# JasonHopeSpace/panda

Measured on AMD Instinct MI355X. Metric: MSM points/s (BN254, 2^24), higher is better.
Workload: dtype u32; 1 GPU; BN254 MSM 2^24 points per GPU, Jacobian output, bases and scalars resident in HBM; curve=bn254, log_points_per_gpu=24, exchange=none

## Files before the change

### panda_amd/csrc/msm_sort.hip

```cpp
#include <algorithm>
#include <atomic>
#include <cmath>

#include "fe29.h"
#include "msm_sort.h"

using namespace panda29;

namespace {

constexpr unsigned SORT_TILE = 8192;
constexpr unsigned MAX_PARTS = 1024;
constexpr unsigned SORT_THREADS = 1024;
constexpr unsigned BS_CHUNK = 8192;

template <class Code>
struct CodeTraits;
template <>
struct CodeTraits<uint16_t> {
    static constexpr u32 ZERO = 0x7fffu;
    static constexpr u32 MAG = 0x7fffu;
    static constexpr int SIGN = 15;
};
template <>
struct CodeTraits<u32> {
    static constexpr u32 ZERO = 0x7fffffffu;
    static constexpr u32 MAG = 0x7fffffffu;
    static constexpr int SIGN = 31;
};

template <int WORDS>
__device__ __forceinline__ void load_words(u32 *dst, const u32 *src)
{
    static_assert(WORDS % 4 == 0, "vector loads");
    const uint4 *s4 = reinterpret_cast<const uint4 *>(src);
#pragma unroll
    for (int i = 0; i < WORDS / 4; i++) {
        uint4 v = s4[i];
        dst[4 * i] = v.x;
        dst[4 * i + 1] = v.y;
        dst[4 * i + 2] = v.z;
        dst[4 * i + 3] = v.w;
    }
}

__device__ __forceinline__ void check_samples(const panda::SampleCheck &sc)
{
    int differs = 0;
    for (unsigned t = threadIdx.x >> 2; t < panda::REG_SAMPLES; t += blockDim.x >> 2) {
        const u64 row = panda::sample_row(t, sc.n);
        for (unsigned k = threadIdx.x & 3u; k < sc.row_words; k += 4) differs |= sc.samples[t * sc.row_words + k] != sc.wire[row * sc.row_words + k];
    }
    differs = __syncthreads_or(differs);
    if (threadIdx.x == 0) {
        *sc.flag_dev = differs ? 1u : 0u;
        if (differs) *sc.flag_host = 1u;
    }
}

struct DigitsBatch {
    unsigned log_n, prefix_bit;
};

__device__ __forceinline__ void stage_plan(u32 *wlo, const panda::WindowPlan &plan)
{
    for (unsigned k = threadIdx.x; k < plan.W; k += blockDim.x) wlo[k] = plan.lo[k] | ((u32)plan.width[k] << 16);
}

template <int L, class CT, class Fn>
__device__ __forceinline__ void for_each_digit(const u32 *s, const u32 *wlo, unsigned W, u32 prefix, Fn f)
{
    u32 carry = 0;
    unsigned k = 0;
    auto digit = [&](u32 raw, unsigned c) {
        const u32 half = 1u << (c - 1), full = 1u << c;
        raw += carry;
        u32 code;
        if (raw >= half) {
            u32 mag = full - raw;
            carry = 1;
            code = mag ? ((1u << CT::SIGN) | prefix | (mag - 1)) : CT::ZERO;
        } else {
            carry = 0;
            code = raw ? (prefix | (raw - 1)) : CT::ZERO;
        }
        f(k, code);
    };
#pragma unroll
    for (int m = 0; m < L; m++) {
        const u64 v = s[m] | ((u64)s[m + 1] << 32);
        while (k < W) {
            const u32 e = __builtin_amdgcn_readfirstlane(wlo[k]);
            const unsigned lo = e & 0xffffu, c = e >> 16;
            if ((lo >> 5) != (unsigned)m) break;
            digit((u32)(v >> (lo & 31)) & ((1u << c) - 1), c);
            k++;
        }
    }
    for (; k < W; k++) digit(0, __builtin_amdgcn_readfirstlane(wlo[k]) >> 16);
}

template <class Fr, class Code, bool BATCH = false>
__global__ void __launch_bounds__(256) k_digits(const u32 *__restrict__ scalars, Code *__restrict__ dig, u64 n, panda::WindowPlan plan, panda::SampleCheck sc,
                                                DigitsBatch bg)
{
    typedef CodeTraits<Code> CT;
    constexpr int L = Fr::L;
    __shared__ u32 wlo[panda::MAX_WINDOWS];
    if (blockIdx.x == 0 && sc.wire) check_samples(sc);
    stage_plan(wlo, plan);
    __syncthreads();
    u64 i = (u64)blockIdx.x * blockDim.x + threadIdx.x;
    if (i >= n) return;
    u32 w[L], s[L + 1];
    load_words<L>(w, scalars + i * L);
    fe_wire_to_canonical<Fr>(s, w);
    s[L] = 0;
    const u32 prefix = BATCH ? (u32)(i >> bg.log_n) << bg.prefix_bit : 0u;
    for_each_digit<L, CT>(s, wlo, plan.W, prefix, [&](unsigned k, u32 code) { dig[(u64)k * n + i] = (Code)code; });
}

struct DigitsHistGeom {
    unsigned lo_bits, H, tiles;
};

template <class Fr, class Code, bool BATCH = false>
__global__ void __launch_bounds__(1024) k_digits_hist(const u32 *__restrict__ scalars, Code *__restrict__ dig, u32 *__restrict__ tile_hist, u64 n,
                                                     panda::WindowPlan plan, DigitsHistGeom g, panda::SampleCheck sc, DigitsBatch bg)
{
    typedef CodeTraits<Code> CT;
    constexpr int L = Fr::L;
    extern __shared__ u32 hist[];
    __shared__ u32 wlo[panda::MAX_WINDOWS];
    if (blockIdx.x == 0 && sc.wire) check_samples(sc);
    const unsigned tile = blockIdx.x, tid = threadIdx.x;
    const unsigned WH = plan.W * g.H, threads = blockDim.x;
    for (unsigned i = tid; i < WH; i += threads) hist[i] = 0;
    stage_plan(wlo, plan);
    __syncthreads();
    const u64 begin = (u64)tile * SORT_TILE, end = begin + SORT_TILE < n ? begin + SORT_TILE : n;
    u32 w[L];
    if (begin + tid < end) load_words<L>(w, scalars + (begin + tid) * L);
    for (u64 i = begin + tid; i < end; i += threads) {
        u32 s[L + 1];
        fe_wire_to_canonical<Fr>(s, w);
        if (i + threads < end) load_words<L>(w, scalars + (i + threads) * L);
        s[L] = 0;
        const u32 prefix = BATCH ? (u32)(i >> bg.log_n) << bg.prefix_bit : 0u;
        for_each_digit<L, CT>(s, wlo, plan.W, prefix, [&](unsigned k, u32 code) {
            dig[(u64)k * n + i] = (Code)code;
            if (code != CT::ZERO) atomicAdd(&hist[k * g.H + ((code & CT::MAG) >> g.lo_bits)], 1u);
        });
    }
    __syncthreads();
    for (unsigned i = tid; i < WH; i += threads) {
        const unsigned k = i / g.H, h = i - k * g.H;
        tile_hist[((u64)k * g.tiles + tile) * g.H + h] = hist[i];
    }
}

template <class Code, class Fn>
__device__ __forceinline__ void for_each_code(const Code *__restrict__ dw, u64 begin, u64 end, Fn f)
{
    constexpr unsigned PER = 16 / sizeof(Code);
    if (reinterpret_cast<uintptr_t>(dw + begin) & 15) {
        for (u64 a = begin + threadIdx.x; a < end; a += blockDim.x) f(a, (u32)dw[a]);
        return;
    }
    for (u64 a = begin + (u64)threadIdx.x * PER; a < end; a += (u64)blockDim.x * PER) {
        const uint4 v = *reinterpret_cast<const uint4 *>(dw + a);
        const u32 wv[4] = {v.x, v.y, v.z, v.w};
#pragma unroll
        for (unsigned j = 0; j < PER; j++) {
            const u32 code = sizeof(Code) == 2 ? (wv[j >> 1] >> (16 * (j & 1))) & 0xffffu : wv[j];
            if (a + j < end) f(a + j, code);
        }
    }
}


struct SortGeom {
    unsigned log_n, lo_bits, H, tiles;
    u32 row0;
};

template <class Code>
__global__ void __launch_bounds__(256) k_part_hist(const Code *__restrict__ dig, u32 *__restrict__ tile_hist, SortGeom g)
{
    typedef CodeTraits<Code> CT;
    __shared__ u32 h[MAX_PARTS];
    const unsigned w = blockIdx.y, tile = blockIdx.x, tid = threadIdx.x;
    for (unsigned i = tid; i < g.H; i += 256) h[i] = 0;
    __syncthreads();
    const u64 n = (u64)1 << g.log_n;
    const Code *dw = dig + ((u64)w << g.log_n);
    const u64 begin = (u64)tile * SORT_TILE, end = begin + SORT_TILE < n ? begin + SORT_TILE : n;
    for_each_code<Code>(dw, begin, end, [&](u64, u32 code) {
        if (code != CT::ZERO) atomicAdd(&h[(code & CT::MAG) >> g.lo_bits], 1u);
    });
    __syncthreads();
    u32 *out = tile_hist + ((u64)w * g.tiles + tile) * g.H;
    for (unsigned i = tid; i < g.H; i += 256) out[i] = h[i];
}

__global__ void __launch_bounds__(1024) k_part_scan_cols(const u32 *__restrict__ tile_hist, u32 *__restrict__ tile_pref, u32 *__restrict__ totals, SortGeom g)
{
    const unsigned w = blockIdx.y, lane = threadIdx.x & 63, h = blockIdx.x * 16 + (threadIdx.x >> 6);
    if (h >= g.H) return;
    const u64 col = (u64)w * g.tiles * g.H + h;
    u32 run = 0;
    for (unsigned t0 = 0; t0 < g.tiles; t0 += 64) {
        const unsigned tile = t0 + lane;
        u32 v = tile < g.tiles ? tile_hist[col + (u64)tile * g.H] : 0;
        u32 inc = v;
        for (unsigned d = 1; d < 64; d <<= 1) {
            u32 up = __shfl_up(inc, d, 64);
            if (lane >= d) inc += up;
        }
        if (tile < g.tiles) tile_pref[col + (u64)tile * g.H] = run + inc - v;
        run += __shfl(inc, 63, 64);
    }
    if (lane == 0) totals[(u64)w * g.H + h] = run;
}

__device__ __forceinline__ u32 block_inclusive_scan(u32 v, u32 *wsum)
{
    const unsigned lane = threadIdx.x & 63u, wave = threadIdx.x >> 6;
    for (unsigned d = 1; d < 64; d <<= 1) {
        const u32 up = __shfl_up(v, d, 64);
        if (lane >= d) v += up;
    }
    if (lane == 63) wsum[wave] = v;
    __syncthreads();
    for (unsigned w = 0; w < wave; w++) v += wsum[w];
    return v;
}

__global__ void __launch_bounds__(1024) k_part_offsets(const u32 *__restrict__ totals, u32 *__restrict__ part_off, SortGeom g)
{
    __shared__ u32 wsum[16];
    const unsigned w = blockIdx.x, t = threadIdx.x;
    const u32 mine = t < g.H ? totals[(u64)w * g.H + t] : 0;
    const u32 inc = block_inclusive_scan(mine, wsum);
    if (t < g.H) part_off[(u64)w * (g.H + 1) + t] = inc - mine;
    if (t == 1023) part_off[(u64)w * (g.H + 1) + g.H] = inc;
}

template <class Code, unsigned THREADS>
struct TileCodes {
    static constexpr unsigned PER = 16 / sizeof(Code), LOADS = SORT_TILE / (THREADS * PER);
    static_assert(LOADS * THREADS * PER == SORT_TILE, "whole loads");
    uint4 v[LOADS];
    bool vec;
    __device__ __forceinline__ void load(const Code *__restrict__ dw, u64 begin, u64 end)
    {
        vec = !(reinterpret_cast<uintptr_t>(dw + begin) & 15);
        if (!vec) return;
#pragma unroll
        for (unsigned q = 0; q < LOADS; q++) {
            const u64 a = begin + ((u64)q * THREADS + threadIdx.x) * PER;
            v[q] = a < end ? *reinterpret_cast<const uint4 *>(dw + a) : uint4{0, 0, 0, 0};
        }
    }
    __device__ __forceinline__ u32 code(unsigned q, unsigned j) const
    {
        const u32 wv[4] = {v[q].x, v[q].y, v[q].z, v[q].w};
        return sizeof(Code) == 2 ? (wv[j >> 1] >> (16 * (j & 1))) & 0xffffu : wv[j];
    }
    template <class Rank, class Place>
    __device__ __forceinline__ void rank_and_place(const Code *__restrict__ dw, u64 begin, u64 end, Rank rank, Place place) const
    {
        if (!vec) {
            for_each_code<Code>(dw, begin, end, [&](u64 i, u32 c) { place(i, c, rank(i, c)); });
            return;
        }
        u32 slot[LOADS * PER];
#pragma unroll
        for (unsigned q = 0; q < LOADS; q++) {
            const u64 a = begin + ((u64)q * THREADS + threadIdx.x) * PER;
#pragma unroll
            for (unsigned j = 0; j < PER; j++)
                if (a + j < end) slot[q * PER + j] = rank(a + j, code(q, j));
        }
#pragma unroll
        for (unsigned q = 0; q < LOADS; q++) {
            const u64 a = begin + ((u64)q * THREADS + threadIdx.x) * PER;
#pragma unroll
            for (unsigned j = 0; j < PER; j++)
                if (a + j < end) place(a + j, code(q, j), slot[q * PER + j]);
        }
    }
};

template <class Code, class Word>
__global__ void __launch_bounds__(SORT_THREADS) k_part_scatter(const Code *__restrict__ dig, const u32 *__restrict__ tile_hist, const u32 *__restrict__ tile_pref,
                                                      const u32 *__restrict__ part_off, Word *__restrict__ p1, SortGeom g)
{
    typedef CodeTraits<Code> CT;
    static_assert(MAX_PARTS <= SORT_THREADS, "a partition counter per thread");
    __shared__ u32 lcur[MAX_PARTS];
    __shared__ u32 delta[MAX_PARTS];
    __shared__ Word words[SORT_TILE];
    __shared__ uint16_t parts_of[SORT_TILE];
    __shared__ u32 wsum[SORT_THREADS / 64];
    const unsigned w = blockIdx.y, tile = blockIdx.x, tid = threadIdx.x;
    const u64 row = ((u64)w * g.tiles + tile) * g.H;
    const u32 *po = part_off + (u64)w * (g.H + 1);
    const u64 n = (u64)1 << g.log_n;
    const Code *dw = dig + ((u64)w << g.log_n);
    Word *pw = p1 + ((u64)w << g.log_n);
    const u64 begin = (u64)tile * SORT_TILE, end = begin + SORT_TILE < n ? begin + SORT_TILE : n;
    const u32 lo_mask = (1u << g.lo_bits) - 1;
    TileCodes<Code, SORT_THREADS> codes;
    codes.load(dw, begin, end);
    const u32 count = tid < g.H ? tile_hist[row + tid] : 0;
    const u32 gbase = tid < g.H ? po[tid] + tile_pref[row + tid] : 0;
    const u32 lstart = block_inclusive_scan(count, wsum) - count;
    if (tid < g.H) {
        lcur[tid] = lstart;
        delta[tid] = gbase - lstart;
    }
    __syncthreads();
    codes.rank_and_place(
        dw, begin, end, [&](u64, u32 code) -> u32 { return code == CT::ZERO ? 0u : atomicAdd(&lcur[(code & CT::MAG) >> g.lo_bits], 1u); },
        [&](u64 i, u32 code, u32 slot) {
            if (code == CT::ZERO) return;
            u32 b = code & CT::MAG, h = b >> g.lo_bits;
            words[slot] = ((Word)(b & lo_mask) << (g.log_n + 1)) | (Word)(((code >> CT::SIGN) << g.log_n) | (u32)i);
            parts_of[slot] = (uint16_t)h;
        });
    __syncthreads();
    const u32 total = lcur[g.H - 1];
    for (u32 j = tid; j < total; j += SORT_THREADS) pw[delta[parts_of[j]] + j] = words[j];
}

template <class Code>
__global__ void __launch_bounds__(SORT_THREADS) k1_scatter_split(const Code *__restrict__ dig, const u32 *__restrict__ tile_hist, const u32 *__restrict__ tile_pref,
                                                        const u32 *__restrict__ part_off, u32 *__restrict__ p1_lo, unsigned char *__restrict__ p1_hi, SortGeom g,
                                                        unsigned b3)
{
    typedef CodeTraits<Code> CT;
    static_assert(MAX_PARTS <= SORT_THREADS, "a partition counter per thread");
    __shared__ u32 lcur[MAX_PARTS];
    __shared__ u32 delta[MAX_PARTS];
    __shared__ u32 words[SORT_TILE];
    __shared__ u32 meta[SORT_TILE];
    __shared__ u32 wsum[SORT_THREADS / 64];
    const unsigned w = blockIdx.y, tile = blockIdx.x, tid = threadIdx.x, lane = tid & 63u;
    const u64 row = ((u64)w * g.tiles + tile) * g.H;
    const u32 *po = part_off + (u64)w * (g.H + 1);
    const u64 n = (u64)1 << g.log_n;
    const Code *dw = dig + ((u64)w << g.log_n);
    u32 *plo = p1_lo + ((u64)w << g.log_n);
    unsigned char *phi = p1_hi + ((u64)w << g.log_n);
    const u64 begin = (u64)tile * SORT_TILE, end = begin + SORT_TILE < n ? begin + SORT_TILE : n;
    const u32 b3_mask = (1u << b3) - 1, b2_mask = (1u << (g.lo_bits - b3)) - 1;
    TileCodes<Code, SORT_THREADS> codes;
    codes.load(dw, begin, end);
    const u32 count = tid < g.H ? tile_hist[row + tid] : 0;
    const u32 gbase = tid < g.H ? po[tid] + tile_pref[row + tid] : 0;
    const u32 lstart = block_inclusive_scan(count, wsum) - count;
    if (tid < g.H) {
        lcur[tid] = lstart;
        delta[tid] = gbase - lstart;
    }
    __syncthreads();
    codes.rank_and_place(
        dw, begin, end, [&](u64, u32 code) -> u32 { return code == CT::ZERO ? 0u : atomicAdd(&lcur[(code & CT::MAG) >> g.lo_bits], 1u); },
        [&](u64 i, u32 code, u32 slot) {
            if (code == CT::ZERO) return;
            u32 b = code & CT::MAG, h = b >> g.lo_bits;
            words[slot] = ((b & b3_mask) << (g.log_n + 1)) | ((code >> CT::SIGN) << g.log_n) | (u32)i;
            meta[slot] = (h << 8) | ((b >> b3) & b2_mask);
        });
    __syncthreads();
    const u32 total = lcur[g.H - 1];
    for (u32 base = 0; base < total; base += SORT_THREADS) {
        const u32 j = base + tid;
        const bool valid = j < total;
        const u32 m = valid ? meta[j] : ~0u;
        const u32 h = m >> 8;
        u32 dst = 0;
        if (valid) {
            dst = delta[h] + j;
            plo[dst] = words[j];
        }
        const u32 m1 = __shfl_down(m, 1, 64), m2 = __shfl_down(m, 2, 64), m3 = __shfl_down(m, 3, 64);
        const bool lead = valid && lane <= 60 && !(reinterpret_cast<uintptr_t>(phi + dst) & 3) && (m1 >> 8) == h && (m2 >> 8) == h && (m3 >> 8) == h;
        const u64 leaders = __ballot(lead);
        const bool covered = (((leaders << 1) | (leaders << 2) | (leaders << 3)) >> lane) & 1;
        if (lead)
            *reinterpret_cast<u32 *>(phi + dst) = (m & 0xffu) | ((m1 & 0xffu) << 8) | ((m2 & 0xffu) << 16) | (m3 << 24);
        else if (valid && !covered)
            phi[dst] = (unsigned char)m;
    }
}

__device__ __forceinline__ void scan128_inclusive(u32 *cnt, u32 *carry )
{
    const unsigned tid = threadIdx.x, lane = tid & 63u;
    u32 v = tid < 128 ? cnt[tid] : 0;
    if (tid < 128) {
        for (unsigned d = 1; d < 64; d <<= 1) {
            const u32 up = __shfl_up(v, d, 64);
            if (lane >= d) v += up;
        }
        if (tid == 63) *carry = v;
    }
    __syncthreads();
    if (tid >= 64 && tid < 128) v += *carry;
    if (tid < 128) cnt[tid] = v;
    __syncthreads();
}

__global__ void __launch_bounds__(SORT_THREADS) k_bucket_sort(const u32 *__restrict__ p1, const u32 *__restrict__ part_off, u32 *__restrict__ off,
                                                     u32 *__restrict__ sorted, SortGeom g, unsigned NB)
{
    __shared__ u32 cnt[128], cur[128], lstart[128], lcur[128], scan_carry;
    __shared__ u32 words[BS_CHUNK];
    __shared__ unsigned char lo_of[BS_CHUNK];
    const unsigned w = blockIdx.y, h = blockIdx.x, tid = threadIdx.x;
    const unsigned L = 1u << g.lo_bits;
    const u32 ps = part_off[(u64)w * (g.H + 1) + h], pe = part_off[(u64)w * (g.H + 1) + h + 1];
    const u32 *pw = p1 + ((u64)w << g.log_n);
    u32 *sw = sorted + ((u64)w << g.log_n);
    const unsigned shift = g.log_n + 1;
    if (tid < 128) cnt[tid] = 0;
    __syncthreads();
    for (u32 j = ps + tid; j < pe; j += SORT_THREADS) atomicAdd(&cnt[pw[j] >> shift], 1u);
    __syncthreads();
    u32 mine = tid < 128 ? cnt[tid] : 0;
    scan128_inclusive(cnt, &scan_carry);
    if (tid < L) {
        u32 start = ps + cnt[tid] - mine;
        cur[tid] = start;
        off[(u64)w * (NB + 1) + ((u64)h << g.lo_bits) + tid] = start;
    }
    if (h == g.H - 1 && tid == 0) off[(u64)w * (NB + 1) + NB] = pe;
    __syncthreads();
    const u32 id_mask = (1u << g.log_n) - 1;
    for (u32 cbeg = ps; cbeg < pe; cbeg += BS_CHUNK) {
        const u32 cend = min(cbeg + BS_CHUNK, pe);
        if (tid < 128) {
            lstart[tid] = 0;
            lcur[tid] = 0;
        }
        __syncthreads();
        for (u32 j = cbeg + tid; j < cend; j += SORT_THREADS) atomicAdd(&lstart[pw[j] >> shift], 1u);
        __syncthreads();
        u32 c0 = tid < 128 ? lstart[tid] : 0;
        scan128_inclusive(lstart, &scan_carry);
        if (tid < 128) {
            lstart[tid] -= c0;
            cnt[tid] = c0;
        }
        __syncthreads();
        for (u32 j = cbeg + tid; j < cend; j += SORT_THREADS) {
            u32 v = pw[j];
            u32 l = v >> shift;
            u32 slot = lstart[l] + atomicAdd(&lcur[l], 1u);
            words[slot] = ((v & id_mask) + g.row0) | (((v >> g.log_n) & 1u) << 31);
            lo_of[slot] = (unsigned char)l;
        }
        __syncthreads();
        for (u32 j = tid; j < cend - cbeg; j += SORT_THREADS) {
            u32 l = lo_of[j];
            sw[cur[l] + (j - lstart[l])] = words[j];
        }
        __syncthreads();
        if (tid < 128) cur[tid] += cnt[tid];
        __syncthreads();
    }
}


struct TabledGeom {
    unsigned log_n, W;
    unsigned b1, b2, b3;
    unsigned H1, H2, S;
    unsigned max_tiles2;
    unsigned Q;
    unsigned row_shift;
    u32 row0;
    unsigned per_window;
    u32 row_mask;
};
__host__ __device__ __forceinline__ unsigned seg_of(const TabledGeom &g, unsigned k, unsigned h1) { return h1 * g.W + k; }

struct SortRange {
    unsigned s_lo, s_hi, q_lo, q_hi;
};

__global__ void __launch_bounds__(SORT_THREADS) k2_seg_tiles(const u32 *__restrict__ part_off, u32 *__restrict__ seg_tile, TabledGeom g)
{
    __shared__ u32 wsum[SORT_THREADS / 64];
    const unsigned tid = threadIdx.x;
    const unsigned per = (g.S + SORT_THREADS - 1) / SORT_THREADS;
    u32 local = 0;
    for (unsigned j = 0; j < per; j++) {
        unsigned s = tid * per + j;
        if (s < g.S) {
            unsigned k = s % g.W, h1 = s / g.W;
            const u32 *po = part_off + (u64)k * (g.H1 + 1);
            local += (po[h1 + 1] - po[h1] + SORT_TILE - 1) / SORT_TILE;
        }
    }
    const u32 inc = block_inclusive_scan(local, wsum);
    u32 run = inc - local;
    for (unsigned j = 0; j < per; j++) {
        unsigned s = tid * per + j;
        if (s < g.S) {
            unsigned k = s % g.W, h1 = s / g.W;
            const u32 *po = part_off + (u64)k * (g.H1 + 1);
            seg_tile[s] = run;
            run += (po[h1 + 1] - po[h1] + SORT_TILE - 1) / SORT_TILE;
        }
    }
    if (tid == SORT_THREADS - 1) seg_tile[g.S] = inc;
}

struct TileRange {
    unsigned s;
    u64 begin, end;
    u64 seg_begin;
};

__device__ __forceinline__ bool locate_tile(TileRange &r, unsigned &tile, unsigned rel, const u32 *seg_tile, const u32 *part_off, const TabledGeom &g, const SortRange &R)
{
    tile = seg_tile[R.s_lo] + rel;
    if (tile >= seg_tile[R.s_hi]) return false;
    unsigned lo = R.s_lo, hi = R.s_hi;
    while (hi - lo > 1) {
        unsigned mid = (lo + hi) >> 1;
        if (seg_tile[mid] <= tile) lo = mid;
        else hi = mid;
    }
    r.s = lo;
    const unsigned k = lo % g.W, h1 = lo / g.W;
    const u32 *po = part_off + (u64)k * (g.H1 + 1);
    r.seg_begin = ((u64)k << g.log_n) + po[h1];
    const u64 seg_end = ((u64)k << g.log_n) + po[h1 + 1];
    r.begin = r.seg_begin + (u64)(tile - seg_tile[lo]) * SORT_TILE;
    r.end = r.begin + SORT_TILE < seg_end ? r.begin + SORT_TILE : seg_end;
    return true;
}

__global__ void __launch_bounds__(256) k2_hist(const unsigned char *__restrict__ p1_hi, const u32 *__restrict__ part_off, const u32 *__restrict__ seg_tile,
                                               u32 *__restrict__ tile_hist, TabledGeom g, SortRange R)
{
    __builtin_amdgcn_s_setprio(3);
    __shared__ u32 h[256];
    const unsigned tid = threadIdx.x;
    unsigned tile;
    TileRange r;
    if (!locate_tile(r, tile, blockIdx.x, seg_tile, part_off, g, R)) return;
    h[tid] = 0;
    __syncthreads();
    const u64 first = r.begin & ~(u64)15;
    for (u64 a = first + (u64)tid * 16; a < r.end; a += 256 * 16) {
        const uint4 v = *reinterpret_cast<const uint4 *>(p1_hi + a);
        const u32 wv[4] = {v.x, v.y, v.z, v.w};
#pragma unroll
        for (int j = 0; j < 16; j++) {
            const u64 i = a + j;
            if (i >= r.begin && i < r.end) atomicAdd(&h[(wv[j >> 2] >> (8 * (j & 3))) & 0xffu], 1u);
        }
    }
    __syncthreads();
    if (tid < g.H2) tile_hist[(u64)tile * g.H2 + tid] = h[tid];
}

__global__ void __launch_bounds__(256) k2_scan_cols(const u32 *__restrict__ tile_hist, u32 *__restrict__ tile_pref, const u32 *__restrict__ seg_tile,
                                                    u32 *__restrict__ totals, TabledGeom g, SortRange R)
{
    __builtin_amdgcn_s_setprio(3);
    const unsigned s = R.s_lo + blockIdx.y, lane = threadIdx.x & 63, h = blockIdx.x * 4 + (threadIdx.x >> 6);
    if (h >= g.H2) return;
    const unsigned t_begin = seg_tile[s], t_end = seg_tile[s + 1];
    u32 run = 0;
    for (unsigned t0 = t_begin; t0 < t_end; t0 += 64) {
        const unsigned tile = t0 + lane;
        u32 v = tile < t_end ? tile_hist[(u64)tile * g.H2 + h] : 0;
        u32 inc = v;
        for (unsigned d = 1; d < 64; d <<= 1) {
            u32 up = __shfl_up(inc, d, 64);
            if (lane >= d) inc += up;
        }
        if (tile < t_end) tile_pref[(u64)tile * g.H2 + h] = run + inc - v;
        run += __shfl(inc, 63, 64);
    }
    if (lane == 0) totals[(u64)s * g.H2 + h] = run;
}

__global__ void __launch_bounds__(256) k2_offsets(const u32 *__restrict__ totals, u32 *__restrict__ sub_off, TabledGeom g, SortRange R)
{
    __builtin_amdgcn_s_setprio(3);
    __shared__ u32 wsum[4];
    const unsigned s = R.s_lo + blockIdx.x, t = threadIdx.x;
    const u32 mine = t < g.H2 ? totals[(u64)s * g.H2 + t] : 0;
    const u32 inc = block_inclusive_scan(mine, wsum);
    if (t < g.H2) sub_off[(u64)s * (g.H2 + 1) + t] = inc - mine;
    if (t == 255) sub_off[(u64)s * (g.H2 + 1) + g.H2] = inc;
}

template <unsigned THREADS>
__global__ void __launch_bounds__(THREADS) k2_scatter(const u32 *__restrict__ p1_lo, const unsigned char *__restrict__ p1_hi, const u32 *__restrict__ part_off,
                                                  const u32 *__restrict__ seg_tile, const u32 *__restrict__ tile_hist, const u32 *__restrict__ tile_pref,
                                                  const u32 *__restrict__ sub_off, u32 *__restrict__ p2, TabledGeom g, SortRange R)
{
    __builtin_amdgcn_s_setprio(3);
    __shared__ u32 lcur[256];
    __shared__ u32 delta[256];
    __shared__ u32 words[SORT_TILE];
    __shared__ unsigned char parts_of[SORT_TILE];
    __shared__ u32 wsum[THREADS / 64];
    static_assert(THREADS >= 256, "a sub-partition counter per thread");
    const unsigned tid = threadIdx.x;
    unsigned tile;
    TileRange r;
    if (!locate_tile(r, tile, blockIdx.x, seg_tile, part_off, g, R)) return;
    const u64 first = r.begin & ~(u64)7, a0 = first + (u64)tid * 8;
    uint2 kv{0, 0};
    uint4 w0{0, 0, 0, 0}, w1{0, 0, 0, 0};
    if (a0 < r.end) {
        kv = *reinterpret_cast<const uint2 *>(p1_hi + a0);
        w0 = *reinterpret_cast<const uint4 *>(p1_lo + a0);
        w1 = *reinterpret_cast<const uint4 *>(p1_lo + a0 + 4);
    }
    const u32 count = tid < g.H2 ? tile_hist[(u64)tile * g.H2 + tid] : 0;
    const u32 gbase = tid < g.H2 ? (u32)r.seg_begin + sub_off[(u64)r.s * (g.H2 + 1) + tid] + tile_pref[(u64)tile * g.H2 + tid] : 0;
    const u32 lstart = block_inclusive_scan(count, wsum) - count;
    if (tid < g.H2) {
        lcur[tid] = lstart;
        delta[tid] = gbase - lstart;
    }
    __syncthreads();
    for (u64 a = a0; a < r.end; a += (u64)THREADS * 8) {
        if (a != a0) {
            kv = *reinterpret_cast<const uint2 *>(p1_hi + a);
            w0 = *reinterpret_cast<const uint4 *>(p1_lo + a);
            w1 = *reinterpret_cast<const uint4 *>(p1_lo + a + 4);
        }
        const u32 keys[2] = {kv.x, kv.y};
        const u32 ws[8] = {w0.x, w0.y, w0.z, w0.w, w1.x, w1.y, w1.z, w1.w};
        u32 slot[8];
#pragma unroll
        for (int j = 0; j < 8; j++) {
            const u64 i = a + j;
            if (i >= r.begin && i < r.end) slot[j] = atomicAdd(&lcur[(keys[j >> 2] >> (8 * (j & 3))) & 0xffu], 1u);
        }
#pragma unroll
        for (int j = 0; j < 8; j++) {
            const u64 i = a + j;
            if (i >= r.begin && i < r.end) {
                words[slot[j]] = ws[j];
                parts_of[slot[j]] = (unsigned char)((keys[j >> 2] >> (8 * (j & 3))) & 0xffu);
            }
        }
    }
    __syncthreads();
    const u32 total = (u32)(r.end - r.begin);
    for (u32 j = tid; j < total; j += THREADS) p2[delta[parts_of[j]] + j] = words[j];
}


__device__ __forceinline__ void cell_run(u64 &begin, u32 &len, unsigned k, unsigned h1, unsigned h2, const u32 *part_off, const u32 *sub_off, const TabledGeom &g)
{
    const unsigned s = seg_of(g, k, h1);
    const u32 *so = sub_off + (u64)s * (g.H2 + 1);
    begin = ((u64)k << g.log_n) + part_off[(u64)k * (g.H1 + 1) + h1] + so[h2];
    len = so[h2 + 1] - so[h2];
}

__device__ __forceinline__ unsigned cells_total(const TabledGeom &g) { return g.per_window ? g.W * g.Q : g.Q; }

__global__ void __launch_bounds__(1024) k3_cell_counts(const u32 *__restrict__ sub_off, u32 *__restrict__ cell_cnt, u32 *__restrict__ blk_sum, TabledGeom g, SortRange R)
{
    __builtin_amdgcn_s_setprio(3);
    __shared__ u32 red[16];
    const unsigned blk = R.q_lo / 1024 + blockIdx.x, t = threadIdx.x;
    const unsigned qbits = g.b1 + g.b2;
    u32 sum = 0;
#pragma unroll 1
    for (unsigned q = blk * 1024 + t; q < blk * 1024 + 1024 && q < R.q_hi; q += blockDim.x) {
        const unsigned cell = g.per_window ? q & ((1u << qbits) - 1) : q;
        const unsigned h1 = cell >> g.b2, h2 = cell & (g.H2 - 1);
        const unsigned k_begin = g.per_window ? q >> qbits : 0u, k_end = g.per_window ? k_begin + 1 : g.W;
        u32 total = 0;
#pragma unroll 1
        for (unsigned k = k_begin; k < k_end; k++) {
            const unsigned at = seg_of(g, k, h1) * (g.H2 + 1) + h2;
            total += sub_off[at + 1] - sub_off[at];
        }
        cell_cnt[q] = total;
        sum += total;
    }
    for (unsigned d = 32; d > 0; d >>= 1) sum += __shfl_down(sum, d, 64);
    if ((t & 63) == 0) red[t >> 6] = sum;
    __syncthreads();
    if (t == 0) {
        u32 v = 0;
        for (unsigned i = 0; i < blockDim.x / 64; i++) v += red[i];
        blk_sum[blk] = v;
    }
}

__global__ void __launch_bounds__(1024) k3_cell_offsets(const u32 *__restrict__ cell_cnt, const u32 *__restrict__ blk_sum, u32 *__restrict__ cell_off, TabledGeom g, SortRange R)
{
    __builtin_amdgcn_s_setprio(3);
    __shared__ u32 wsum[16], wsum_before[16], before;
    const unsigned blk = R.q_lo / 1024 + blockIdx.x, t = threadIdx.x, T = blockDim.x, per = 1024 / T;
    u32 v = 0;
    for (unsigned b = t; b < blk; b += T) v += blk_sum[b];
    const unsigned q0 = blk * 1024 + t * per;
    u32 local = 0;
    for (unsigned j = 0; j < per; j++) local += q0 + j < R.q_hi ? cell_cnt[q0 + j] : 0;
    v = block_inclusive_scan(v, wsum_before);
    if (t == T - 1) before = v;
    const u32 inc = block_inclusive_scan(local, wsum);
    u32 run = before + inc - local;
    for (unsigned j = 0; j < per; j++) {
        const unsigned q = q0 + j;
        if (q < R.q_hi) {
            cell_off[q] = run;
            run += cell_cnt[q];
            if (q == R.q_hi - 1) cell_off[R.q_hi] = run;
        }
    }
}

constexpr unsigned K3_THREADS = 1024;
constexpr unsigned K3_PER = 16;
constexpr unsigned K3_CAP = K3_THREADS * K3_PER;
constexpr unsigned K3_PER_WIDE = 32;

#ifdef PANDA_K3_STAMPS
__device__ unsigned long long g_k3_stamps[1024 * 8];
#define K3_STAMP(n)                                                                                                          \
    do {                                                                                                                     \
        if (threadIdx.x == 0 && (cell & 15u) == 0 && (cell >> 4) < 1024) g_k3_stamps[(cell >> 4) * 8 + (n)] = __builtin_amdgcn_s_memrealtime(); \
    } while (0)
#else
#define K3_STAMP(n)
#endif

template <unsigned PER, unsigned THREADS = K3_THREADS, bool BATCH = false>
__global__ void __launch_bounds__(THREADS) k3_merge(const u32 *__restrict__ p2, const u32 *__restrict__ part_off, const u32 *__restrict__ sub_off,
                                              const u32 *__restrict__ cell_off, u32 *__restrict__ off, u32 *__restrict__ sorted, TabledGeom g, unsigned NB, SortRange R)
{
    __shared__ u32 cnt[128], cur[128], scan_carry;
    constexpr unsigned IMG = THREADS * K3_PER;
    __shared__ u32 outbuf[IMG];
    __shared__ u64 rbegin[64];
    __shared__ u32 vstart[65];
    const unsigned tid = threadIdx.x;
    const unsigned cell = R.q_lo + blockIdx.x;
    const unsigned k0 = g.per_window ? cell / g.Q : 0u, q = g.per_window ? cell % g.Q : cell;
    const unsigned nruns = g.per_window ? 1u : g.W;
    const unsigned h1 = q / g.H2, h2 = q % g.H2;
    const unsigned L = 1u << g.b3;
    K3_STAMP(0);
    const u32 out_rel = cell_off[cell] - (g.per_window ? cell_off[k0 * g.Q] : 0u);
    const bool closes_part = !g.per_window && cell + 1 == R.q_hi && q + 1 < g.Q;
    u32 *sw = sorted + ((u64)k0 << g.log_n);
    u32 *ow = off + (u64)k0 * (NB + 1);
    if (tid < 64) {
        u64 b = 0;
        u32 len = 0;
        if (tid < nruns) {
            cell_run(b, len, k0 + tid, h1, h2, part_off, sub_off, g);
            rbegin[tid] = b;
        }
        u32 inc = len;
// ... 317 lines not shown

static bool sort3_supported(unsigned log_n, const WindowPlan &plan, bool per_window, unsigned group_log = 0);
static size_t sort3_bytes(unsigned log_n, const WindowPlan &plan, bool per_window, unsigned group_log = 0);
static hipError_t sort3(hipStream_t stream, Arena &arena, unsigned fr, const void *scalars, unsigned log_n, const WindowPlan &plan, SortEvents ev, SortResult *out,
                        SortPlacement place, SampleCheck check, bool per_window, SortSplit *split = nullptr, unsigned group_log = 0);

bool msm_sort_plain_supported(unsigned log_n, const WindowPlan &plan)
{
    const unsigned c = plan.width[0];
    if (c <= 16) return c >= 2 && plain_geom(log_n, c).H <= MAX_PARTS;
    return sort3_supported(log_n, plan, true);
}

size_t msm_sort_plain_bytes(unsigned log_n, const WindowPlan &plan)
{
    if (plan.width[0] > 16) return sort3_bytes(log_n, plan, true);
    const u64 n = (u64)1 << log_n;
    const unsigned W = plan.W, c = plan.width[0], NB = 1u << (c - 1);
    const SortGeom g = plain_geom(log_n, c);
    return align256(n * W * 2 + 16) + 2 * align256((size_t)W * g.tiles * g.H * 4) + 2 * align256((size_t)W * (g.H + 1) * 4) + align256((size_t)W * (NB + 1) * 4) +
           2 * align256(n * W * 4) + 4096;
}

hipError_t msm_sort_plain(hipStream_t stream, Arena &arena, unsigned fr, const void *scalars, unsigned log_n, const WindowPlan &plan, SortEvents ev,
                          SortResult *out, SortPlacement place, SampleCheck check)
{
    if (plan.width[0] > 16) return sort3(stream, arena, fr, scalars, log_n, plan, ev, out, place, check, true);
    const u64 n = (u64)1 << log_n;
    const unsigned W = plan.W, c = plan.width[0], NB = 1u << (c - 1);
    if (c < 2) return hipErrorInvalidValue;
    SortGeom geom = plain_geom(log_n, c);
    if (geom.H > MAX_PARTS) return hipErrorInvalidValue;
    if (place.row_shift) {
        if ((u64)place.row0 + n > ((u64)1 << 31)) return hipErrorInvalidValue;
        geom.row0 = place.row0;
    }
    uint16_t *d_dig = (uint16_t *)arena.take(n * W * 2 + 16);
    u32 *d_thist = (u32 *)arena.take((size_t)W * geom.tiles * geom.H * 4);
    u32 *d_tpref = (u32 *)arena.take((size_t)W * geom.tiles * geom.H * 4);
    u32 *d_poff = (u32 *)arena.take((size_t)W * (geom.H + 1) * 4);
    u32 *d_ptot = (u32 *)arena.take((size_t)W * (geom.H + 1) * 4);
    u32 *d_p1 = (u32 *)arena.take(n * W * 4);
    u32 *d_off = (u32 *)arena.take((size_t)W * (NB + 1) * 4);
    u32 *d_sorted = (u32 *)arena.take(n * W * 4);
    if (!d_dig || !d_thist || !d_tpref || !d_poff || !d_ptot || !d_p1 || !d_off || !d_sorted) return hipErrorOutOfMemory;

    const bool fused = launch_digits_hist_for<uint16_t>(fr, stream, scalars, d_dig, d_thist, n, plan, geom, check);
    if (!fused) launch_digits_for<uint16_t>(fr, stream, scalars, d_dig, n, plan, check);
    if (ev.digits_done) PANDA_TRY(hipEventRecord(ev.digits_done, stream));
    if (!fused) hipLaunchKernelGGL(k_part_hist<uint16_t>, dim3(geom.tiles, W), dim3(256), 0, stream, d_dig, d_thist, geom);
    hipLaunchKernelGGL(k_part_scan_cols, dim3((geom.H + 15) / 16, W), dim3(1024), 0, stream, d_thist, d_tpref, d_ptot, geom);
    hipLaunchKernelGGL(k_part_offsets, dim3(W), dim3(1024), 0, stream, d_ptot, d_poff, geom);
    hipLaunchKernelGGL((k_part_scatter<uint16_t, u32>), dim3(geom.tiles, W), dim3(SORT_THREADS), 0, stream, d_dig, d_thist, d_tpref, d_poff, d_p1, geom);
    if (ev.partition_done) PANDA_TRY(hipEventRecord(ev.partition_done, stream));
    hipLaunchKernelGGL(k_bucket_sort, dim3(geom.H, W), dim3(SORT_THREADS), 0, stream, d_p1, d_poff, d_off, d_sorted, geom, NB);
    out->off = d_off;
    out->sorted = d_sorted;
    out->lists = W;
    out->NB = NB;
    out->stride = n;
    return hipGetLastError();
}

static bool sort3_supported(unsigned log_n, const WindowPlan &plan, bool per_window, unsigned group_log)
{
    const unsigned c = plan.width[0];
    if (plan.W > 32 || plan.W < 1 || c < 4 || c > 24 || log_n > 26 || log_n < 1) return false;
    if (group_log && (per_window || group_log >= log_n)) return false;
    unsigned wbits = 0;
    while ((1u << wbits) < plan.W) wbits++;
    if (log_n + wbits > 31) return false;
    const TabledGeom g = tabled_geom(log_n, plan, c - 1 + group_log, per_window);
    return g.b1 <= 10 && g.b2 <= 8 && g.b3 <= 7 && g.S <= 16384 && g.b3 + 1 + log_n <= 32;
}

static size_t sort3_bytes(unsigned log_n, const WindowPlan &plan, bool per_window, unsigned group_log)
{
    const u64 E = (u64)plan.W << log_n;
    const unsigned NB = 1u << (plan.width[0] - 1 + group_log);
    const TabledGeom g = tabled_geom(log_n, plan, plan.width[0] - 1 + group_log, per_window);
    const unsigned tiles1 = (unsigned)((((u64)1 << log_n) + SORT_TILE - 1) / SORT_TILE);
    const size_t cells = (size_t)g.Q * (per_window ? g.W : 1u), lists = per_window ? g.W : 1u;
    return align256(E * 4 + 16) + 2 * align256((size_t)g.W * tiles1 * g.H1 * 4) + 2 * align256((size_t)g.W * (g.H1 + 1) * 4) + align256(E * 4 + 64) + align256(E + 16) +
           align256((size_t)(g.S + 1) * 4) + 2 * align256((size_t)g.max_tiles2 * g.H2 * 4) + align256((size_t)g.S * g.H2 * 4) +
           align256((size_t)g.S * (g.H2 + 1) * 4) + align256(E * 4) + 2 * align256((cells + 1) * 4) + align256((cells / 1024 + 1) * 4) +
           align256(lists * (NB + 1) * 4) + align256(E * 4) + 8192;
}

static std::atomic<unsigned> g_wide_merge{0};

static hipError_t sort3(hipStream_t stream, Arena &arena, unsigned fr, const void *scalars, unsigned log_n, const WindowPlan &plan, SortEvents ev, SortResult *out,
                        SortPlacement place, SampleCheck check, bool per_window, SortSplit *split, unsigned group_log)
{
    if (!sort3_supported(log_n, plan, per_window, group_log)) return hipErrorInvalidValue;
    if (group_log && (place.row_shift || split)) return hipErrorInvalidValue;
    const u64 n = (u64)1 << log_n;
    const u64 E = (u64)plan.W << log_n;
    const unsigned W = plan.W, NB = 1u << (plan.width[0] - 1 + group_log);
    TabledGeom g = tabled_geom(log_n, plan, plan.width[0] - 1 + group_log, per_window);
    const DigitsBatch batch{log_n - group_log, plan.width[0] - 1u};
    const DigitsBatch *batch_p = group_log ? &batch : nullptr;
    if (group_log) {
        g.row_shift = log_n - group_log;
        g.row_mask = (1u << (log_n - group_log)) - 1;
    }
    if (place.row_shift) {
        if (place.row_shift < log_n || place.row_shift > 26) return hipErrorInvalidValue;
        const u64 last_row = (per_window ? 0 : ((u64)(W - 1) << place.row_shift)) + place.row0 + n;
        if (last_row > ((u64)1 << 31)) return hipErrorInvalidValue;
        g.row_shift = place.row_shift;
        g.row0 = place.row0;
    }
    SortGeom g1;
    g1.row0 = 0;
    g1.log_n = log_n;
    g1.lo_bits = g.b2 + g.b3;
    g1.H = g.H1;
    g1.tiles = (unsigned)((n + SORT_TILE - 1) / SORT_TILE);
    const unsigned cells = g.Q * (per_window ? W : 1u), lists = per_window ? W : 1u;
    const unsigned qblocks = (cells + 1023) / 1024;

    u32 *d_dig = (u32 *)arena.take(E * 4 + 16);
    u32 *d_thist1 = (u32 *)arena.take((size_t)W * g1.tiles * g.H1 * 4);
    u32 *d_tpref1 = (u32 *)arena.take((size_t)W * g1.tiles * g.H1 * 4);
    u32 *d_poff = (u32 *)arena.take((size_t)W * (g.H1 + 1) * 4);
    u32 *d_ptot = (u32 *)arena.take((size_t)W * (g.H1 + 1) * 4);
    u32 *d_p1_lo = (u32 *)arena.take(E * 4 + 64);
    unsigned char *d_p1_hi = (unsigned char *)arena.take(E + 16);
    u32 *d_segtile = (u32 *)arena.take((size_t)(g.S + 1) * 4);
    u32 *d_thist2 = (u32 *)arena.take((size_t)g.max_tiles2 * g.H2 * 4);
    u32 *d_tpref2 = (u32 *)arena.take((size_t)g.max_tiles2 * g.H2 * 4);
    u32 *d_tot2 = (u32 *)arena.take((size_t)g.S * g.H2 * 4);
    u32 *d_suboff = (u32 *)arena.take((size_t)g.S * (g.H2 + 1) * 4);
    u32 *d_p2 = (u32 *)arena.take(E * 4);
    u32 *d_cellcnt = (u32 *)arena.take((size_t)cells * 4);
    u32 *d_blksum = (u32 *)arena.take((size_t)qblocks * 4);
    u32 *d_celloff = (u32 *)arena.take((size_t)(cells + 1) * 4);
    u32 *d_off = (u32 *)arena.take((size_t)lists * (NB + 1) * 4);
    u32 *d_sorted = (u32 *)arena.take(E * 4);
    if (!d_dig || !d_thist1 || !d_tpref1 || !d_tpref2 || !d_poff || !d_ptot || !d_p1_lo || !d_p1_hi || !d_segtile || !d_thist2 || !d_tot2 || !d_suboff || !d_p2 || !d_cellcnt || !d_blksum || !d_celloff ||
        !d_off || !d_sorted)
        return hipErrorOutOfMemory;

    const bool fused = launch_digits_hist_for<u32>(fr, stream, scalars, d_dig, d_thist1, n, plan, g1, check, batch_p);
    if (!fused) launch_digits_for<u32>(fr, stream, scalars, d_dig, n, plan, check, batch_p);
    if (ev.digits_done) PANDA_TRY(hipEventRecord(ev.digits_done, stream));
    if (!fused) hipLaunchKernelGGL(k_part_hist<u32>, dim3(g1.tiles, W), dim3(256), 0, stream, d_dig, d_thist1, g1);
    hipLaunchKernelGGL(k_part_scan_cols, dim3((g1.H + 15) / 16, W), dim3(1024), 0, stream, d_thist1, d_tpref1, d_ptot, g1);
    hipLaunchKernelGGL(k_part_offsets, dim3(W), dim3(1024), 0, stream, d_ptot, d_poff, g1);
    hipLaunchKernelGGL(k1_scatter_split<u32>, dim3(g1.tiles, W), dim3(SORT_THREADS), 0, stream, d_dig, d_thist1, d_tpref1, d_poff, d_p1_lo, d_p1_hi, g1, g.b3);
    hipLaunchKernelGGL(k2_seg_tiles, dim3(1), dim3(SORT_THREADS), 0, stream, d_poff, d_segtile, g);
    auto level2 = [&](hipStream_t s, const SortRange &R) {
        hipLaunchKernelGGL(k2_hist, dim3(g.max_tiles2), dim3(256), 0, s, d_p1_hi, d_poff, d_segtile, d_thist2, g, R);
        hipLaunchKernelGGL(k2_scan_cols, dim3((g.H2 + 3) / 4, R.s_hi - R.s_lo), dim3(256), 0, s, d_thist2, d_tpref2, d_segtile, d_tot2, g, R);
        hipLaunchKernelGGL(k2_offsets, dim3(R.s_hi - R.s_lo), dim3(256), 0, s, d_tot2, d_suboff, g, R);
        if (s == stream)
            hipLaunchKernelGGL(k2_scatter<SORT_THREADS>, dim3(g.max_tiles2), dim3(SORT_THREADS), 0, s, d_p1_lo, d_p1_hi, d_poff, d_segtile, d_thist2, d_tpref2, d_suboff, d_p2, g, R);
        else
            hipLaunchKernelGGL(k2_scatter<256>, dim3(g.max_tiles2), dim3(256), 0, s, d_p1_lo, d_p1_hi, d_poff, d_segtile, d_thist2, d_tpref2, d_suboff, d_p2, g, R);
    };
    auto level3_counts = [&](hipStream_t s, const SortRange &R) {
        hipLaunchKernelGGL(k3_cell_counts, dim3((R.q_hi - R.q_lo + 1023) / 1024), dim3(s == stream ? 1024 : 256), 0, s, d_suboff, d_cellcnt, d_blksum, g, R);
    };
    unsigned wide_cells = 0, small_from = ~0u;
    if (!per_window) {
        const u64 n = (u64)1 << (log_n - group_log);
        double per_bucket = 0;
        unsigned narrow = plan.width[0];
        for (unsigned k = 0; k < plan.W; k++) {
            per_bucket += ldexp((double)n, -(int)(plan.width[k] - 1));
            narrow = std::min(narrow, (unsigned)plan.width[k]);
        }
        const double densest = ldexp(per_bucket, (int)g.b3);
        if (narrow + 1 == plan.width[0] && densest > (double)K3_CAP * 0.8 && densest <= (double)K3_THREADS * K3_PER_WIDE * 0.8) wide_cells = g.Q / 2;
        double sparse_bucket = 0;
        for (unsigned k = 0; k < plan.W; k++)
            if (plan.width[k] == plan.width[0]) sparse_bucket += ldexp((double)n, -(int)(plan.width[k] - 1));
        if (narrow + 1 == plan.width[0] && ldexp(sparse_bucket, (int)g.b3) <= 256.0 * K3_PER * 0.85) small_from = g.Q / 2;
        const bool plan_wide = wide_cells != 0;
        const unsigned mode = g_wide_merge.load(std::memory_order_relaxed);
        if (mode == 1) wide_cells = g.Q, small_from = ~0u;
        if (mode == 2) wide_cells = 0, small_from = ~0u;
        if (mode == 3) wide_cells = 0, small_from = 0;
        if (group_log) wide_cells = plan_wide ? g.Q : 0u, small_from = ~0u;
    }
    auto level3_merge = [&](hipStream_t s, const SortRange &R) {
        hipLaunchKernelGGL(k3_cell_offsets, dim3((R.q_hi - R.q_lo + 1023) / 1024), dim3(s == stream ? 1024 : 256), 0, s, d_cellcnt, d_blksum, d_celloff, g, R);
        if (s == stream) {
            const unsigned wide_hi = std::min(std::max(wide_cells, R.q_lo), R.q_hi);
            if (wide_hi > R.q_lo) {
                const SortRange Rw{R.s_lo, R.s_hi, R.q_lo, wide_hi};
                if (group_log)
                    hipLaunchKernelGGL((k3_merge<K3_PER_WIDE, K3_THREADS, true>), dim3(wide_hi - R.q_lo), dim3(K3_THREADS), 0, s, d_p2, d_poff, d_suboff, d_celloff, d_off, d_sorted, g, NB, Rw);
                else
                    hipLaunchKernelGGL(k3_merge<K3_PER_WIDE>, dim3(wide_hi - R.q_lo), dim3(K3_THREADS), 0, s, d_p2, d_poff, d_suboff, d_celloff, d_off, d_sorted, g, NB, Rw);
            }
            const unsigned small_lo = std::min(std::max(small_from, wide_hi), R.q_hi);
            if (small_lo > wide_hi) {
                const SortRange Rn{R.s_lo, R.s_hi, wide_hi, small_lo};
                if (group_log)
                    hipLaunchKernelGGL((k3_merge<K3_PER, K3_THREADS, true>), dim3(small_lo - wide_hi), dim3(K3_THREADS), 0, s, d_p2, d_poff, d_suboff, d_celloff, d_off, d_sorted, g, NB, Rn);
                else
                    hipLaunchKernelGGL(k3_merge<K3_PER>, dim3(small_lo - wide_hi), dim3(K3_THREADS), 0, s, d_p2, d_poff, d_suboff, d_celloff, d_off, d_sorted, g, NB, Rn);
            }
            if (R.q_hi > small_lo) {
                const SortRange Rs{R.s_lo, R.s_hi, small_lo, R.q_hi};
                hipLaunchKernelGGL((k3_merge<K3_PER, 256>), dim3(R.q_hi - small_lo), dim3(256), 0, s, d_p2, d_poff, d_suboff, d_celloff, d_off, d_sorted, g, NB, Rs);
            }
        } else
            hipLaunchKernelGGL(k3_merge_small<256>, dim3(R.q_hi - R.q_lo), dim3(256), 0, s, d_p2, d_poff, d_suboff, d_celloff, d_off, d_sorted, g, NB, R);
    };
    unsigned cut_h1 = 0;
    if (split) {
        split->active = false;
        const unsigned step = g.H2 >= 1024 ? 1u : 1024u / g.H2;
        if (split->helper && !per_window && split->front_of_128 && g.H1 >= 2 * step && g.Q % 1024 == 0) {
            cut_h1 = (unsigned)(((u64)g.H1 * split->front_of_128 / 128 + step / 2) / step * step);
            cut_h1 = std::min(std::max(cut_h1, step), g.H1 - step);
        }
    }
    if (cut_h1) {
        const SortRange front{0, cut_h1 * W, 0, cut_h1 * g.H2}, rest{cut_h1 * W, g.S, cut_h1 * g.H2, g.Q};
        level2(stream, front);
        if (ev.partition_done) PANDA_TRY(hipEventRecord(ev.partition_done, stream));
        level3_counts(stream, front);
        level3_merge(stream, front);
        PANDA_TRY(hipEventRecord(split->ev_front, stream));
        PANDA_TRY(hipStreamWaitEvent(split->helper, split->ev_front, 0));
        level2(split->helper, rest);
        level3_counts(split->helper, rest);
        level3_merge(split->helper, rest);
        PANDA_TRY(hipEventRecord(split->rest_done, split->helper));
        split->active = true;
        split->pos = d_celloff;
        split->cells = g.Q;
        split->cut_cell = cut_h1 * g.H2;
        split->cut_bucket = split->cut_cell << g.b3;
    } else {
        const SortRange all{0, g.S, 0, cells};
        level2(stream, all);
        if (ev.partition_done) PANDA_TRY(hipEventRecord(ev.partition_done, stream));
        level3_counts(stream, all);
        level3_merge(stream, all);
    }
    out->off = d_off;
    out->sorted = d_sorted;
    out->lists = lists;
    out->NB = NB;
    out->stride = per_window ? n : E;
    return hipGetLastError();
}

#ifdef PANDA_K3_STAMPS
extern "C" int panda_debug_k3_stamps(unsigned long long *out) { return (int)hipMemcpyFromSymbol(out, HIP_SYMBOL(g_k3_stamps), sizeof(unsigned long long) * 1024 * 8); }
#endif
void msm_sort_set_wide_merge(unsigned mode) { g_wide_merge.store(mode, std::memory_order_relaxed); }
bool msm_sort_tabled_supported(unsigned log_n, const WindowPlan &plan) { return sort3_supported(log_n, plan, false); }
size_t msm_sort_tabled_bytes(unsigned log_n, const WindowPlan &plan) { return sort3_bytes(log_n, plan, false); }

bool msm_sort_tabled_batch_supported(unsigned log_n, unsigned group_log, const WindowPlan &plan)
{
    return group_log >= 1 && log_n >= 1 && log_n + group_log <= 26 && sort3_supported(log_n + group_log, plan, false, group_log);
}
size_t msm_sort_tabled_batch_bytes(unsigned log_n, unsigned group_log, const WindowPlan &plan) { return sort3_bytes(log_n + group_log, plan, false, group_log); }
hipError_t msm_sort_tabled_batch(hipStream_t stream, Arena &arena, unsigned fr, const void *scalars, unsigned log_n, unsigned group_log, const WindowPlan &plan,
                                 SortResult *out, SampleCheck check)
{
    if (!msm_sort_tabled_batch_supported(log_n, group_log, plan)) return hipErrorInvalidValue;
    return sort3(stream, arena, fr, scalars, log_n + group_log, plan, SortEvents{nullptr, nullptr}, out, SortPlacement{0, 0}, check, false, nullptr, group_log);
}

hipError_t msm_sort_tabled(hipStream_t stream, Arena &arena, unsigned fr, const void *scalars, unsigned log_n, const WindowPlan &plan, SortEvents ev,
                           SortResult *out, SortPlacement place, SampleCheck check, SortSplit *split)
{
    return sort3(stream, arena, fr, scalars, log_n, plan, ev, out, place, check, false, split);
}

}
```

Before: 953.4 million points/s.

## Vectorize column scans, remap scatter tiles per XCD, prefetch k2_hist loads

Rewrites the level-1 and level-2 column prefix-scan kernels so each lane handles four adjacent histogram columns with vector loads. Tiles are spread across waves (level 1) or the next tile row is prefetched (level 2), which removes the strided single-column accesses. Adds an XCD-aware block-index remap to the scatter kernels so neighbouring tiles run on the same XCD and can share its L2. The level-2 histogram kernel now issues its first two loads before clearing shared memory, and uses predicated atomics instead of branches. These changes touch several unrelated sort stages, and the remap assumes a round-robin dispatch over 8 XCDs.

```diff
diff --git a/panda_amd/csrc/msm_sort.hip b/panda_amd/csrc/msm_sort.hip
--- a/panda_amd/csrc/msm_sort.hip
+++ b/panda_amd/csrc/msm_sort.hip
@@ -4,6 +4,7 @@
 
 #include "fe29.h"
 #include "msm_sort.h"
+#include "xcd_remap.h"
 
 using namespace panda29;
 
@@ -203,24 +204,87 @@
     for (unsigned i = tid; i < g.H; i += 256) out[i] = h[i];
 }
 
+
+__device__ __forceinline__ void load_cols4(u32 *v, const u32 *__restrict__ row, unsigned c, unsigned H, bool vec)
+{
+    if (vec) {
+        const uint4 q = c < H ? *reinterpret_cast<const uint4 *>(row + c) : uint4{0, 0, 0, 0};
+        v[0] = q.x, v[1] = q.y, v[2] = q.z, v[3] = q.w;
+    } else {
+#pragma unroll
+        for (unsigned i = 0; i < 4; i++) v[i] = c + i < H ? row[c + i] : 0;
+    }
+}
+__device__ __forceinline__ void store_cols4(u32 *__restrict__ row, const u32 *v, unsigned c, unsigned H, bool vec)
+{
+    if (vec) {
+        if (c < H) *reinterpret_cast<uint4 *>(row + c) = uint4{v[0], v[1], v[2], v[3]};
+    } else {
+#pragma unroll
+        for (unsigned i = 0; i < 4; i++)
+            if (c + i < H) row[c + i] = v[i];
+    }
+}
+__device__ __forceinline__ void scan_tiles16(u32 *v, unsigned lane)
+{
+#pragma unroll
+    for (unsigned d = 4; d < 64; d <<= 1) {
+#pragma unroll
+        for (unsigned i = 0; i < 4; i++) {
+            const u32 up = __shfl_up(v[i], d, 64);
+            if (lane >= d) v[i] += up;
+        }
+    }
+}
+
 __global__ void __launch_bounds__(1024) k_part_scan_cols(const u32 *__restrict__ tile_hist, u32 *__restrict__ tile_pref, u32 *__restrict__ totals, SortGeom g)
 {
-    const unsigned w = blockIdx.y, lane = threadIdx.x & 63, h = blockIdx.x * 16 + (threadIdx.x >> 6);
-    if (h >= g.H) return;
-    const u64 col = (u64)w * g.tiles * g.H + h;
-    u32 run = 0;
-    for (unsigned t0 = 0; t0 < g.tiles; t0 += 64) {
-        const unsigned tile = t0 + lane;
-        u32 v = tile < g.tiles ? tile_hist[col + (u64)tile * g.H] : 0;
-        u32 inc = v;
-        for (unsigned d = 1; d < 64; d <<= 1) {
-            u32 up = __shfl_up(inc, d, 64);
-            if (lane >= d) inc += up;
-        }
-        if (tile < g.tiles) tile_pref[col + (u64)tile * g.H] = run + inc - v;
-        run += __shfl(inc, 63, 64);
-    }
-    if (lane == 0) totals[(u64)w * g.H + h] = run;
+    __shared__ u32 wtot[16][16];
+    const unsigned w = blockIdx.y, lane = threadIdx.x & 63, wave = threadIdx.x >> 6, ts = lane >> 2, quad = lane & 3u;
+    const unsigned c = blockIdx.x * 16 + 4 * quad;
+    const bool vec = !(g.H & 3u);
+    const u64 base = (u64)w * g.tiles * g.H;
+    const unsigned per = (g.tiles + 255) / 256 * 16;
+    const unsigned t_lo = min(wave * per, g.tiles), t_hi = min(t_lo + per, g.tiles);
+    u32 run[4] = {0, 0, 0, 0}, v[4];
+    for (unsigned t0 = t_lo; t0 < t_hi; t0 += 16) {
+        const unsigned tile = t0 + ts;
+        if (tile < t_hi) {
+            load_cols4(v, tile_hist + base + (u64)tile * g.H, c, g.H, vec);
+#pragma unroll
+            for (unsigned i = 0; i < 4; i++) run[i] += v[i];
+        }
+    }
+#pragma unroll
+    for (unsigned d = 4; d < 64; d <<= 1)
+#pragma unroll
+        for (unsigned i = 0; i < 4; i++) run[i] += __shfl_xor(run[i], d, 64);
+    if (ts == 0)
+#pragma unroll
+        for (unsigned i = 0; i < 4; i++) wtot[wave][4 * quad + i] = run[i];
+    __syncthreads();
+#pragma unroll
+    for (unsigned i = 0; i < 4; i++) {
+        run[i] = 0;
+        for (unsigned j = 0; j < wave; j++) run[i] += wtot[j][4 * quad + i];
+    }
+    for (unsigned t0 = t_lo; t0 < t_hi; t0 += 16) {
+        const unsigned tile = t0 + ts;
+        u32 inc[4] = {0, 0, 0, 0};
+        if (tile < t_hi) load_cols4(inc, tile_hist + base + (u64)tile * g.H, c, g.H, vec);
+#pragma unroll
+        for (unsigned i = 0; i < 4; i++) v[i] = inc[i];
+        scan_tiles16(inc, lane);
+#pragma unroll
+        for (unsigned i = 0; i < 4; i++) v[i] = run[i] + inc[i] - v[i];
+        if (tile < t_hi) store_cols4(tile_pref + base + (u64)tile * g.H, v, c, g.H, vec);
+#pragma unroll
+        for (unsigned i = 0; i < 4; i++) run[i] += __shfl(inc[i], 60 + quad, 64);
+    }
+    if (wave == 15 && ts == 0)
+#pragma unroll
+        for (unsigned i = 0; i < 4; i++)
+            if (c + i < g.H) totals[(u64)w * g.H + c + i] = run[i];
 }
 
 __device__ __forceinline__ u32 block_inclusive_scan(u32 v, u32 *wsum)
@@ -303,7 +367,7 @@
     __shared__ Word words[SORT_TILE];
     __shared__ uint16_t parts_of[SORT_TILE];
     __shared__ u32 wsum[SORT_THREADS / 64];
-    const unsigned w = blockIdx.y, tile = blockIdx.x, tid = threadIdx.x;
+    const unsigned w = blockIdx.y, tile = panda::xcd_remap(blockIdx.x, gridDim.x), tid = threadIdx.x;
     const u64 row = ((u64)w * g.tiles + tile) * g.H;
     const u32 *po = part_off + (u64)w * (g.H + 1);
     const u64 n = (u64)1 << g.log_n;
@@ -346,7 +410,7 @@
     __shared__ u32 words[SORT_TILE];
     __shared__ u32 meta[SORT_TILE];
     __shared__ u32 wsum[SORT_THREADS / 64];
-    const unsigned w = blockIdx.y, tile = blockIdx.x, tid = threadIdx.x, lane = tid & 63u;
+    const unsigned w = blockIdx.y, tile = panda::xcd_remap(blockIdx.x, gridDim.x), tid = threadIdx.x, lane = tid & 63u;
     const u64 row = ((u64)w * g.tiles + tile) * g.H;
     const u32 *po = part_off + (u64)w * (g.H + 1);
     const u64 n = (u64)1 << g.log_n;
@@ -554,18 +618,23 @@
     unsigned tile;
     TileRange r;
     if (!locate_tile(r, tile, blockIdx.x, seg_tile, part_off, g, R)) return;
-    h[tid] = 0;
-    __syncthreads();
-    const u64 first = r.begin & ~(u64)15;
-    for (u64 a = first + (u64)tid * 16; a < r.end; a += 256 * 16) {
-        const uint4 v = *reinterpret_cast<const uint4 *>(p1_hi + a);
+    const u64 first = r.begin & ~(u64)15, a0 = first + (u64)tid * 16;
+    auto count = [&](const uint4 &v, u64 a) {
         const u32 wv[4] = {v.x, v.y, v.z, v.w};
 #pragma unroll
         for (int j = 0; j < 16; j++) {
             const u64 i = a + j;
-            if (i >= r.begin && i < r.end) atomicAdd(&h[(wv[j >> 2] >> (8 * (j & 3))) & 0xffu], 1u);
-        }
-    }
+            atomicAdd(&h[(wv[j >> 2] >> (8 * (j & 3))) & 0xffu], (i >= r.begin && i < r.end) ? 1u : 0u);
+        }
+    };
+    uint4 v0{0, 0, 0, 0}, v1{0, 0, 0, 0};
+    if (a0 < r.end) v0 = *reinterpret_cast<const uint4 *>(p1_hi + a0);
+    if (a0 + 256 * 16 < r.end) v1 = *reinterpret_cast<const uint4 *>(p1_hi + a0 + 256 * 16);
+    h[tid] = 0;
+    __syncthreads();
+    if (a0 < r.end) count(v0, a0);
+    if (a0 + 256 * 16 < r.end) count(v1, a0 + 256 * 16);
+    for (u64 a = a0 + 2 * 256 * 16; a < r.end; a += 256 * 16) count(*reinterpret_cast<const uint4 *>(p1_hi + a), a);
     __syncthreads();
     if (tid < g.H2) tile_hist[(u64)tile * g.H2 + tid] = h[tid];
 }
@@ -574,22 +643,30 @@
                                                     u32 *__restrict__ totals, TabledGeom g, SortRange R)
 {
     __builtin_amdgcn_s_setprio(3);
-    const unsigned s = R.s_lo + blockIdx.y, lane = threadIdx.x & 63, h = blockIdx.x * 4 + (threadIdx.x >> 6);
-    if (h >= g.H2) return;
+    const unsigned s = R.s_lo + blockIdx.y, lane = threadIdx.x & 63, ts = lane >> 2, quad = lane & 3u;
+    const unsigned c0 = (blockIdx.x * 4 + (threadIdx.x >> 6)) * 16, c = c0 + 4 * quad;
+    if (c0 >= g.H2) return;
+    const bool vec = !(g.H2 & 3u);
     const unsigned t_begin = seg_tile[s], t_end = seg_tile[s + 1];
-    u32 run = 0;
-    for (unsigned t0 = t_begin; t0 < t_end; t0 += 64) {
-        const unsigned tile = t0 + lane;
-        u32 v = tile < t_end ? tile_hist[(u64)tile * g.H2 + h] : 0;
-        u32 inc = v;
-        for (unsigned d = 1; d < 64; d <<= 1) {
-            u32 up = __shfl_up(inc, d, 64);
-            if (lane >= d) inc += up;
-        }
-        if (tile < t_end) tile_pref[(u64)tile * g.H2 + h] = run + inc - v;
-        run += __shfl(inc, 63, 64);
-    }
-    if (lane == 0) totals[(u64)s * g.H2 + h] = run;
+    u32 run[4] = {0, 0, 0, 0}, next[4] = {0, 0, 0, 0};
+    if (t_begin + ts < t_end) load_cols4(next, tile_hist + (u64)(t_begin + ts) * g.H2, c, g.H2, vec);
+    for (unsigned t0 = t_begin; t0 < t_end; t0 += 16) {
+        const unsigned tile = t0 + ts;
+        u32 v[4], inc[4];
+#pragma unroll
+        for (unsigned i = 0; i < 4; i++) v[i] = inc[i] = next[i], next[i] = 0;
+        if (tile + 16 < t_end) load_cols4(next, tile_hist + (u64)(tile + 16) * g.H2, c, g.H2, vec);
+        scan_tiles16(inc, lane);
+#pragma unroll
+        for (unsigned i = 0; i < 4; i++) v[i] = run[i] + inc[i] - v[i];
+        if (tile < t_end) store_cols4(tile_pref + (u64)tile * g.H2, v, c, g.H2, vec);
+#pragma unroll
+        for (unsigned i = 0; i < 4; i++) run[i] += __shfl(inc[i], 60 + quad, 64);
+    }
+    if (ts == 0)
+#pragma unroll
+        for (unsigned i = 0; i < 4; i++)
+            if (c + i < g.H2) totals[(u64)s * g.H2 + c + i] = run[i];
 }
 
 __global__ void __launch_bounds__(256) k2_offsets(const u32 *__restrict__ totals, u32 *__restrict__ sub_off, TabledGeom g, SortRange R)
@@ -618,7 +695,9 @@
     const unsigned tid = threadIdx.x;
     unsigned tile;
     TileRange r;
-    if (!locate_tile(r, tile, blockIdx.x, seg_tile, part_off, g, R)) return;
+    const unsigned ntiles = seg_tile[R.s_hi] - seg_tile[R.s_lo];
+    if (blockIdx.x >= ntiles) return;
+    if (!locate_tile(r, tile, panda::xcd_remap(blockIdx.x, ntiles), seg_tile, part_off, g, R)) return;
     const u64 first = r.begin & ~(u64)7, a0 = first + (u64)tid * 8;
     uint2 kv{0, 0};
     uint4 w0{0, 0, 0, 0}, w1{0, 0, 0, 0};
@@ -1242,7 +1321,7 @@
     hipLaunchKernelGGL(k2_seg_tiles, dim3(1), dim3(SORT_THREADS), 0, stream, d_poff, d_segtile, g);
     auto level2 = [&](hipStream_t s, const SortRange &R) {
         hipLaunchKernelGGL(k2_hist, dim3(g.max_tiles2), dim3(256), 0, s, d_p1_hi, d_poff, d_segtile, d_thist2, g, R);
-        hipLaunchKernelGGL(k2_scan_cols, dim3((g.H2 + 3) / 4, R.s_hi - R.s_lo), dim3(256), 0, s, d_thist2, d_tpref2, d_segtile, d_tot2, g, R);
+        hipLaunchKernelGGL(k2_scan_cols, dim3((g.H2 + 63) / 64, R.s_hi - R.s_lo), dim3(256), 0, s, d_thist2, d_tpref2, d_segtile, d_tot2, g, R);
         hipLaunchKernelGGL(k2_offsets, dim3(R.s_hi - R.s_lo), dim3(256), 0, s, d_tot2, d_suboff, g, R);
         if (s == stream)
             hipLaunchKernelGGL(k2_scatter<SORT_THREADS>, dim3(g.max_tiles2), dim3(SORT_THREADS), 0, s, d_p1_lo, d_p1_hi, d_poff, d_segtile, d_thist2, d_tpref2, d_suboff, d_p2, g, R);
diff --git a/panda_amd/csrc/xcd_remap.h b/panda_amd/csrc/xcd_remap.h
--- /dev/null
+++ b/panda_amd/csrc/xcd_remap.h
@@ -0,0 +1,21 @@
+#pragma once
+
+#if defined(__HIPCC__)
+#define PANDA_XCD_HD __host__ __device__ __forceinline__
+#else
+#define PANDA_XCD_HD inline
+#endif
+
+namespace panda {
+
+constexpr unsigned XCDS = 8;
+
+PANDA_XCD_HD unsigned xcd_remap(unsigned id, unsigned nwg)
+{
+    const unsigned cls = id % XCDS, idx = id / XCDS;
+    const unsigned q = nwg / XCDS, r = nwg % XCDS;
+    const unsigned first = cls < r ? cls * (q + 1) : r * (q + 1) + (cls - r) * q;
+    return first + idx;
+}
+
+}
```

Measured after the change: 969.7 million points/s (median of 6 runs). +1.7%, better.
